# telegraphroad/VCNF

Measured on AMD Instinct MI355X. Metric: flow transforms/sec (log_prob + sample), D=64 RQ-spline, batch=1M, higher is better.
Workload: dtype f32 results on fp16x3 split operands: every fp32 operand of a conditioner GEMM travels as hi + lo fp16 halves, three f16 matrix instructions per product (four in the 48- and 16-deep layers), fp32 accumulation; measured against fp64 (tests/test_gpu_gemm_error.py): GEMM error 0.6-0.75x the exact-fp32

## Files before the change

vcnf_amd/csrc/fused_layer_v6.hip:

```cpp
#include <hip/hip_runtime.h>
#include <stdint.h>

#include "../../include/vcnf_hip.h"
#include "rqs_math.hpp"
#include "fused_common.hpp"
#include "rqs_lean.hpp"
#include "split_half.hpp"

#ifndef VCNF_ABL
#define VCNF_ABL 0
#endif
#ifndef VCNF_TIME
#define VCNF_TIME 0
#endif
#ifndef VCNF_AHEAD
#define VCNF_AHEAD 1
#endif
#if VCNF_TIME
#define VCNF_T(I) { const long long t_ = clock64(); tacc[I] += t_ - tlast; tlast = t_; }
#define VCNF_TIME_PARAM , float* tstamps
#define VCNF_TIME_ARG , time_buffer()
#else
#define VCNF_T(I)
#define VCNF_TIME_PARAM
#define VCNF_TIME_ARG
#endif

#define VCNF_SYNC() { __builtin_amdgcn_sched_barrier(0); asm volatile("s_waitcnt lgkmcnt(0)\n\ts_barrier" ::: "memory"); __builtin_amdgcn_sched_barrier(0); }

namespace vcnf {

#if VCNF_TIME
constexpr int kTimeSlots = 24;
static float* time_buffer() {
  static float* buf = nullptr;
  if (!buf && hipMalloc(&buf, 2 * kTimeSlots * sizeof(float)) != hipSuccess) buf = nullptr;
  return buf;
}
extern "C" int vcnf_v6_phase_stamps(float* out) {
  if (!time_buffer() || hipDeviceSynchronize() != hipSuccess) return VCNF_ERR_LAUNCH;
  return hipMemcpy(out, time_buffer(), 2 * kTimeSlots * sizeof(float), hipMemcpyDeviceToHost) == hipSuccess ? VCNF_OK : VCNF_ERR_LAUNCH;
}
#endif

template <int DI, int DT, int C, int H, int NBLK, int K, bool INV>
__global__ __launch_bounds__(512, 2) void fused_rqs_layer_v6_kernel(const FusedArgs a VCNF_TIME_PARAM) {
  static_assert(H == 128 && K == 8, "4 row blocks of 32 over 4 waves; 3 K - 1 = 23 logits: two features per 48 rows");
  static_assert((DI == 16 || DI == 32) && DT == DI && (C == 0 || C == 16), "shape family");
  constexpr int kBlock = 512;
  constexpr int kTile = 128;
  constexpr int NCB = 4;
  constexpr int D = DI + DT;
  constexpr int XS = D + 4;
  constexpr int NTX = DI / 16;
  constexpr int NTC = C / 16;
  constexpr int NT0 = NTX + NTC;
  constexpr int NTH = H / 16;
  constexpr int P = 3 * K - 1;
  constexpr int NG = DT / 4;
  constexpr int NR = NG / 2;
  constexpr int TABW = 3 * (K + 1);
  using L = PackLayout6<DI, DT, C, H, NBLK, K>;
  constexpr int GFRAG = 3 * NTH * 2 * 64;
  constexpr int RING = VCNF_AHEAD + 1;

  extern __shared__ __align__(16) float smem[];
  uint4* act = reinterpret_cast<uint4*>(smem);
  uint4* act_hi = act;
  uint4* act_lo = act + NTH * NCB * 64;
  float* xt = smem + 2 * GFRAG * 4;
  uint4* ctxf = reinterpret_cast<uint4*>(xt + kTile * XS);
  float* tab = reinterpret_cast<float*>(ctxf + (C > 0 ? NCB * 2 * 64 : 0));
  float* ldt = tab + ((DI * TABW + 3) & ~3);
  int* tfi = reinterpret_cast<int*>(ldt + kTile);
  int* idi = tfi + DT;
  constexpr int NBV = C > 0 ? 3 : 2;
  constexpr int NBT = 1 + NBLK * NBV;
  constexpr int BPL = NG * 48 + NBT * (H / 2);
  float* biasf = reinterpret_cast<float*>(idi + DI + 4);
  float* ldold = biasf + 2 * BPL;
  int* tflag = reinterpret_cast<int*>(ldold + kTile);

  const int tid = threadIdx.x;
  const int lane = tid & 63;
  const int wave = __builtin_amdgcn_readfirstlane(tid >> 6);
  const int rp = wave & 3;
  const int ch = wave >> 2;
  const int c32 = lane & 31;
  const int kg = lane >> 5;
  const RqsConst& c = a.c;
  const bool shared = a.sh_w != nullptr;
  const LeanConst lc = make_lean_const(c);

  if (ch == 1) __builtin_amdgcn_s_setprio(1);
  for (int i = tid; i < NG * 96; i += kBlock) {
    const int g = i / 96, hf = i % 96 / 48;
    biasf[hf * BPL + g * 48 + i % 48] = a.wpack[L::BF + i];
  }
  for (int i = tid; i < NBT * H; i += kBlock) {
    const int v = i / H, blk = (v - 1) / NBV, sel = (v - 1) % NBV, r = i % H;
    const int off = v == 0 ? L::B0 : L::BLK0 + blk * L::BLK + (sel == 0 ? L::BA : sel == 1 ? L::BB : L::BC);
    biasf[(r >> 4 & 1) * BPL + NG * 48 + v * (H / 2) + (r >> 5) * 16 + (r & 15)] = a.wpack[off + r];
  }
  for (int i = tid; i < DT; i += kBlock) tfi[i] = a.tf_idx[i];
  for (int i = tid; i < DI; i += kBlock) idi[i] = a.id_idx[i];
  if (shared) {
    for (int i = tid; i < 3 * DI; i += kBlock) {
      const int f = i % DI;
      SplitLogits p{a.sh_w + f * K, a.sh_h + f * K, a.sh_d + f * (K - 1), K, 1.f, c.edge_logit, c.tails};
      rqs_build_table_part_k<K>(p, c, tab + f * TABW, 1, i / DI);
    }
  }

  const __amdgpu_buffer_rsrc_t wr =
      __builtin_amdgcn_make_buffer_rsrc(const_cast<float*>(a.wpack), 0, a.wpack_bytes, 0x00020000);
  const int voff = lane * 16;
  const float* bplane = biasf + kg * BPL;

  const long long ntiles = (a.B + kTile - 1) / kTile;
  bool bad = false;
  float satm = 0.f;
#if VCNF_TIME
  long long tacc[20], tlast = clock64();
  const long long tstart = tlast, rstart = wall_clock64();
  for (int i = 0; i < 20; ++i) tacc[i] = 0;
#endif
  float4 xpre[kTile * (D / 4) / kBlock], cpre[1];
  static_assert(kTile * (D / 4) % kBlock == 0 && (C == 0 || kTile * (C / 4) == kBlock), "rows per thread");
#define VCNF_PREFETCH_ROWS(TILE)                                                          \
  {                                                                                       \
    const long long pb0 = min((TILE) * kTile, a.B);                                       \
    const long long left = (a.B - pb0) * (D * 4);                                         \
    const __amdgpu_buffer_rsrc_t xr_ = __builtin_amdgcn_make_buffer_rsrc(                 \
        const_cast<float*>(a.x) + pb0 * D, 0, (int)min(left, (long long)(kTile * D * 4)), 0x00020000); \
    _Pragma("unroll") for (int k = 0; k < kTile * (D / 4) / kBlock; ++k)                  \
      xpre[k] = __builtin_bit_cast(float4, __builtin_amdgcn_raw_buffer_load_b128(xr_, (tid + kBlock * k) * 16, 0, 0)); \
    if (C > 0) {                                                                          \
      const long long leftc = (a.B - pb0) * (C * 4);                                      \
      const __amdgpu_buffer_rsrc_t cr_ = __builtin_amdgcn_make_buffer_rsrc(               \
          const_cast<float*>(a.ctx) + pb0 * C, 0, (int)min(leftc, (long long)(kTile * C * 4)), 0x00020000); \
      cpre[0] = __builtin_bit_cast(float4, __builtin_amdgcn_raw_buffer_load_b128(cr_, tid * 16, 0, 0)); \
    }                                                                                     \
  }
#define VCNF_ROWS_ARRIVED()                                                               \
  {                                                                                       \
    _Pragma("unroll") for (int k = 0; k < kTile * (D / 4) / kBlock; ++k) {                \
      floatx4 v_ = __builtin_bit_cast(floatx4, xpre[k]);                                  \
      asm volatile("" : "+v"(v_));                                                        \
      xpre[k] = __builtin_bit_cast(float4, v_);                                           \
    }                                                                                     \
    if (C > 0) {                                                                          \
      floatx4 v_ = __builtin_bit_cast(floatx4, cpre[0]);                                  \
      asm volatile("" : "+v"(v_));                                                        \
      cpre[0] = __builtin_bit_cast(float4, v_);                                           \
    }                                                                                     \
  }
  VCNF_PREFETCH_ROWS((long long)blockIdx.x)
  VCNF_ROWS_ARRIVED()
  for (long long tile = blockIdx.x; tile < ntiles; tile += gridDim.x) {
    const long long b0 = tile * kTile;
    const int rows = (int)min((long long)kTile, a.B - b0);
    satm = 0.f;
    { VCNF_T(0) VCNF_SYNC(); VCNF_T(15) }
    {
      constexpr int D4 = D / 4;
      if (tid == 0) *tflag = 0;
#pragma unroll
      for (int k = 0; k < kTile * D4 / kBlock; ++k) {
        const int i = tid + kBlock * k;
        const int r = i / D4, o = i - r * D4;
        *reinterpret_cast<float4*>(xt + r * XS + 4 * o) = xpre[k];
      }
      if (C > 0) {
        const int r = tid >> 2, part = tid & 3;
        half4 h4, l4;
        const float cv[4] = {cpre[0].x, cpre[0].y, cpre[0].z, cpre[0].w};
#pragma unroll
        for (int i = 0; i < 4; ++i) satm = fmaxf(satm, cv[i] == cv[i] ? __builtin_fabsf(cv[i]) : __builtin_inff());
        asm volatile("" : "+v"(satm));
#pragma unroll
        for (int i = 0; i < 4; ++i) {
          const float x = __builtin_amdgcn_fmed3f(cv[i], -65504.f, 65504.f);
          const _Float16 hv = (_Float16)x;
          h4[i] = hv;
          l4[i] = (_Float16)((x - (float)hv) * kLoScale);
        }
        const int at = (((r >> 5) * 2) * 64 + (r & 31) + 32 * (part >> 1));
        uint2* dh = reinterpret_cast<uint2*>(ctxf + at) + (part & 1);
        uint2* dl = reinterpret_cast<uint2*>(ctxf + at + 64) + (part & 1);
        *dh = __builtin_bit_cast(uint2, h4);
        *dl = __builtin_bit_cast(uint2, l4);
      }
    }
    { VCNF_T(1) VCNF_SYNC(); VCNF_T(15) }

    {
      constexpr int UNR = DI / 4;
      const int mi = tid >> 2, part = tid & 3;
      float lsum = 0.f;
      float xv[UNR], fv[UNR];
      float* px[UNR];
#pragma unroll
      for (int k = 0; k < UNR; ++k) {
        px[k] = xt + mi * XS + idi[part * UNR + k];
        xv[k] = *px[k];
        fv[k] = xv[k];
      }
      if (shared) {
        float yv[UNR], lad[UNR];
        bool in_[UNR];
#pragma unroll
        for (int k = 0; k < UNR; ++k) {
          in_[k] = (xv[k] >= c.lo_x) && (xv[k] <= c.hi_x);
          bool bad1 = false;
          rqs_point_table_inside<INV, K>(in_[k] ? xv[k] : c.lo_x, tab + (part * UNR + k) * TABW, yv[k], lad[k], bad1);
          bad = bad || (bad1 && in_[k]);
        }
#pragma unroll
        for (int k = 0; k < UNR; ++k) {
          const float o = in_[k] ? yv[k] : xv[k];
          *px[k] = o;
          if (INV) fv[k] = o;
          lsum += in_[k] ? lad[k] : 0.f;
        }
      }
      lsum += __shfl_xor(lsum, 1, 64);
      lsum += __shfl_xor(lsum, 2, 64);
      int tid_ = tid;
      asm volatile("" : "+v"(tid_));
      if (part == 0) ldt[tid_ >> 2] = lsum;
#pragma unroll
      for (int k = 0; k < UNR; ++k) satm = fmaxf(satm, fv[k] == fv[k] ? 0.f : __builtin_inff());
      const int k0 = part * UNR;
      const int t0 = k0 >> 4, kg0 = (k0 >> 3) & 1;
      const int at = (t0 * NCB + (mi >> 5)) * 64 + (mi & 31) + 32 * kg0;
      if (UNR == 8) {
        half8 h8, l8;
        float f8[8];
#pragma unroll
        for (int k = 0; k < 8; ++k) f8[k] = fv[k < UNR ? k : 0];
        split8<false>(f8, h8, l8, satm);
        act_hi[at] = __builtin_bit_cast(uint4, h8);
        act_lo[at] = __builtin_bit_cast(uint4, l8);
      } else {
        half4 h4, l4;
        satm = fmaxf(fmaxf(satm, __builtin_fabsf(fv[0])), __builtin_fabsf(fv[1]));
        satm = fmaxf(fmaxf(satm, __builtin_fabsf(fv[2 < UNR ? 2 : 0])), __builtin_fabsf(fv[3 < UNR ? 3 : 0]));
        asm volatile("" : "+v"(satm));
#pragma unroll
        for (int i = 0; i < 4; ++i) {
          const float x = __builtin_amdgcn_fmed3f(fv[i < UNR ? i : 0], -65504.f, 65504.f);
          const _Float16 hv = (_Float16)x;
          h4[i] = hv;
          l4[i] = (_Float16)((x - (float)hv) * kLoScale);
        }
        reinterpret_cast<uint2*>(act_hi + at)[(k0 >> 2) & 1] = __builtin_bit_cast(uint2, h4);
        reinterpret_cast<uint2*>(act_lo + at)[(k0 >> 2) & 1] = __builtin_bit_cast(uint2, l4);
      }
    }
    { VCNF_T(2) VCNF_SYNC(); VCNF_T(15) }
    if (ch == 1) { VCNF_T(14) VCNF_SYNC(); VCNF_T(16) }

    half8 ahi[NTH], alo[NTH];
    floatx16 abias;
#define VCNF_LOAD_BIAS16(DST, VEC)                                                        \
  _Pragma("unroll") for (int i_ = 0; i_ < 4; ++i_) {                                      \
    const floatx4 b4_ = *reinterpret_cast<const floatx4*>(bplane + NG * 48 + (VEC) * (H / 2) + 16 * rp + 4 * i_); \
    DST[4 * i_ + 0] = b4_[0]; DST[4 * i_ + 1] = b4_[1]; DST[4 * i_ + 2] = b4_[2]; DST[4 * i_ + 3] = b4_[3]; \
  }
#define VCNF_LOAD_HIDDEN(WOFF, BVEC)                                                      \
  {                                                                                       \
    _Pragma("unroll") for (int t = 0; t < NTH; ++t) {                                     \
      ahi[t] = __builtin_bit_cast(half8, wload(wr, voff, 4 * ((WOFF) + ((rp * NTH + t) * 2 + 0) * 256))); \
      alo[t] = __builtin_bit_cast(half8, wload(wr, voff, 4 * ((WOFF) + ((rp * NTH + t) * 2 + 1) * 256))); \
    }                                                                                     \
    VCNF_LOAD_BIAS16(abias, BVEC)                                                         \
  }

    floatx16 h[2];
    {
      half8 w0h[NT0], w0l[NT0];
      floatx16 bias0;
#pragma unroll
      for (int t = 0; t < NT0; ++t) {
        w0h[t] = __builtin_bit_cast(half8, wload(wr, voff, 4 * (L::W0 + ((rp * NT0 + t) * 2 + 0) * 256)));
        w0l[t] = __builtin_bit_cast(half8, wload(wr, voff, 4 * (L::W0 + ((rp * NT0 + t) * 2 + 1) * 256)));
      }
      VCNF_LOAD_BIAS16(bias0, 0)
#pragma unroll
      for (int j = 0; j < 2; ++j) {
        const int cb = 2 * ch + j;
        floatx16 mainv = bias0, corr = {}, corr2 = {};
#pragma unroll
        for (int t = 0; t < NT0; ++t) {
          const half8 bh = __builtin_bit_cast(half8, t < NTX ? act_hi[(t * NCB + cb) * 64 + lane] : ctxf[(cb * 2 + 0) * 64 + lane]);
          const half8 bl = __builtin_bit_cast(half8, t < NTX ? act_lo[(t * NCB + cb) * 64 + lane] : ctxf[(cb * 2 + 1) * 64 + lane]);
          mainv = mfma32h(w0h[t], bh, mainv);
          corr = mfma32h(w0h[t], bl, corr);
          corr = mfma32h(w0l[t], bh, corr);
          corr2 = mfma32h(w0l[t], bl, corr2);
        }
#pragma unroll
        for (int r = 0; r < 16; ++r) h[j][r] = fmaf(fmaf(corr2[r], kLoUnscale, corr[r]), kLoUnscale, mainv[r]);
      }
    }
    { VCNF_T(3) VCNF_SYNC(); VCNF_T(15) }
#define VCNF_PUBLISH(SRC, RELU)                                                           \
  _Pragma("unroll") for (int j = 0; j < 2; ++j) {                                         \
    _Pragma("unroll") for (int hh = 0; hh < 2; ++hh) {                                    \
      float v8_[8];                                                                       \
      _Pragma("unroll") for (int i = 0; i < 8; ++i) v8_[i] = SRC[j][8 * hh + i];          \
      half8 h8_, l8_;                                                                     \
      split8<RELU>(v8_, h8_, l8_, satm);                                                  \
      const int at = ((2 * rp + hh) * NCB + 2 * ch + j) * 64 + lane;                      \
      act_hi[at] = __builtin_bit_cast(uint4, h8_);                                        \
      act_lo[at] = __builtin_bit_cast(uint4, l8_);                                        \
    }                                                                                     \
  }
    VCNF_LOAD_HIDDEN(L::BLK0 + L::WA, 1)
    VCNF_PUBLISH(h, true)
    { VCNF_T(4) VCNF_SYNC(); VCNF_T(15) }

#define VCNF_READ_B(T)                                                                    \
  {                                                                                       \
    rh[(T) % RING] = __builtin_bit_cast(half8, act_hi[((((T) & 7)) * NCB + 2 * ch + ((T) >> 3)) * 64 + lane]); \
    rl[(T) % RING] = __builtin_bit_cast(half8, act_lo[((((T) & 7)) * NCB + 2 * ch + ((T) >> 3)) * 64 + lane]); \
  }
#define VCNF_HIDDEN_COMPUTE(OUT)                                                          \
  {                                                                                       \
    half8 rh[RING], rl[RING];                 \
    floatx16 corr;                                                                        \
    _Pragma("unroll") for (int st_ = 0; st_ < VCNF_AHEAD; ++st_) {                        \
      VCNF_READ_B(st_)                                                                    \
    }                                                                                     \
    _Pragma("unroll") for (int st_ = 0; st_ < 2 * NTH; ++st_) {                           \
      const int j = st_ >> 3, tk_ = st_ & 7;                                              \
      if (st_ + VCNF_AHEAD < 2 * NTH) {                                                   \
        VCNF_READ_B(st_ + VCNF_AHEAD)                                                     \
      }                                                                                   \
      if (tk_ == 0) {                                                                       \
        OUT[j] = abias;                                                                   \
        corr = floatx16{};                                                                \
      }                                                                                   \
      OUT[j] = mfma32h(ahi[tk_], rh[st_ % RING], OUT[j]);                                      \
      corr = mfma32h(ahi[tk_], rl[st_ % RING], corr);                                          \
      corr = mfma32h(alo[tk_], rh[st_ % RING], corr);                                          \
      if (tk_ == NTH - 1) {                                                                 \
        _Pragma("unroll") for (int r = 0; r < 16; ++r) OUT[j][r] = fmaf(corr[r], kLoUnscale, OUT[j][r]); \
      }                                                                                   \
    }                                                                                     \
    __builtin_amdgcn_sched_group_barrier(0x100, 2 * VCNF_AHEAD, 0);                       \
    _Pragma("unroll") for (int st_ = 0; st_ + VCNF_AHEAD < 2 * NTH; ++st_) {              \
      __builtin_amdgcn_sched_group_barrier(0x100, 2, 0);                                  \
      __builtin_amdgcn_sched_group_barrier(0x008, 3, 0);                                  \
    }                                                                                     \
    __builtin_amdgcn_sched_group_barrier(0x008, 3 * VCNF_AHEAD, 0);                       \
  }

#pragma unroll
    for (int blk = 0; blk < (VCNF_ABL == 5 ? 0 : NBLK); ++blk) {
      const int base = L::BLK0 + blk * L::BLK;
      floatx16 t[2];
      VCNF_HIDDEN_COMPUTE(t)
      { VCNF_T(5) VCNF_SYNC(); VCNF_T(15) }
      VCNF_LOAD_HIDDEN(base + L::WB, 2 + blk * NBV)
      half8 wch, wcl;
      floatx16 gate[2], gbias;
      if (C > 0) {
        wch = __builtin_bit_cast(half8, wload(wr, voff, 4 * (base + L::WC + (rp * 2 + 0) * 256)));
        wcl = __builtin_bit_cast(half8, wload(wr, voff, 4 * (base + L::WC + (rp * 2 + 1) * 256)));
        VCNF_LOAD_BIAS16(gbias, 3 + blk * NBV)
      }
      VCNF_PUBLISH(t, true)
      { VCNF_T(6) VCNF_SYNC(); VCNF_T(15) }
      VCNF_HIDDEN_COMPUTE(t)
      if (C > 0 && VCNF_ABL != 6) {
#pragma unroll
        for (int j = 0; j < 2; ++j) {
          const half8 bh = __builtin_bit_cast(half8, ctxf[((2 * ch + j) * 2 + 0) * 64 + lane]);
          const half8 bl = __builtin_bit_cast(half8, ctxf[((2 * ch + j) * 2 + 1) * 64 + lane]);
          floatx16 corr = {}, corr2 = {};
          gate[j] = mfma32h(wch, bh, gbias);
          corr = mfma32h(wch, bl, corr);
          corr = mfma32h(wcl, bh, corr);
          corr2 = mfma32h(wcl, bl, corr2);
#pragma unroll
          for (int r = 0; r < 16; ++r) gate[j][r] = fmaf(fmaf(corr2[r], kLoUnscale, corr[r]), kLoUnscale, gate[j][r]);
        }
      }
      { VCNF_T(5) VCNF_SYNC(); VCNF_T(15) }
      if (blk + 1 < NBLK) {
        VCNF_LOAD_HIDDEN(base + L::BLK + L::WA, 1 + (blk + 1) * NBV)
      }
      if (C > 0 && VCNF_ABL != 6) {
#pragma unroll
        for (int j = 0; j < 2; ++j) {
#pragma unroll
          for (int r = 0; r < 16; ++r) {
            const float sg = hw_rcp(1.f + hw_exp2(-gate[j][r]));
            h[j][r] = fmaf(t[j][r], sg, h[j][r]);
          }
        }
      } else {
#pragma unroll
        for (int j = 0; j < 2; ++j) h[j] += t[j];
      }
      if (blk + 1 < NBLK) {
        VCNF_PUBLISH(h, true)
      } else {
        VCNF_PUBLISH(h, false)
      }
      { VCNF_T(7) VCNF_SYNC(); VCNF_T(15) }
    }
    if (ch == 0) { VCNF_T(14) VCNF_SYNC(); VCNF_T(17) }
#undef VCNF_HIDDEN_COMPUTE
#undef VCNF_READ_B
#undef VCNF_LOAD_HIDDEN
#undef VCNF_PUBLISH

    half8 fhi[NTH], flo[NTH];
#pragma unroll
    for (int t = 0; t < NTH; ++t) {
      fhi[t] = __builtin_bit_cast(half8, act_hi[(t * NCB + rp) * 64 + lane]);
      flo[t] = __builtin_bit_cast(half8, act_lo[(t * NCB + rp) * 64 + lane]);
    }
    float ld_acc = 0.f;
    uint4* win = act + ch * GFRAG;
    const int gtid = tid & 255;
    constexpr int NSTG = GFRAG / 256;
    static_assert(GFRAG % 256 == 0, "whole fragments per thread");
#define VCNF_STAGE_DMA(G)                                                                 \
  _Pragma("unroll") for (int k = 0; k < NSTG; ++k)                                        \
    dma16_to_lds(wr, win + (gtid & ~63) + k * 256, gtid * 16, 4 * (L::WF + (G) * (4 * GFRAG) + k * 1024));
    floatx16 pa[3];
#define VCNF_LOAD_BIASF(G)                                                                \
  _Pragma("unroll") for (int b = 0; b < 3; ++b) {                                         \
    _Pragma("unroll") for (int i_ = 0; i_ < 4; ++i_) {                                    \
      const floatx4 b4_ = *reinterpret_cast<const floatx4*>(bplane + (G) * 48 + 16 * b + 4 * i_); \
      pa[b][4 * i_ + 0] = b4_[0]; pa[b][4 * i_ + 1] = b4_[1]; pa[b][4 * i_ + 2] = b4_[2]; pa[b][4 * i_ + 3] = b4_[3]; \
    }                                                                                     \
  }
    VCNF_LOAD_BIASF(ch)
    { VCNF_T(8) VCNF_SYNC(); VCNF_T(15) }
    VCNF_STAGE_DMA(ch)
    if (ch == 0 && rp < 2 && a.ld_mode) {
      const __amdgpu_buffer_rsrc_t or_ = __builtin_amdgcn_make_buffer_rsrc(a.logdet + b0, 0, rows * 4, 0x00020000);
      __builtin_amdgcn_raw_ptr_buffer_load_lds(or_, (__attribute__((address_space(3))) void*)(ldold + rp * 64), 4,
                                               lane * 4, rp * 256, 0, 0);
    }
    wait_vector_memory();
    { VCNF_T(9) VCNF_SYNC(); VCNF_T(15) }
    if (ch == 1) { VCNF_T(14) VCNF_SYNC(); VCNF_T(18) }
    for (int rnd = 0; rnd < (VCNF_ABL == 3 ? 0 : NR); ++rnd) {
      const int g = 2 * rnd + ch;
      float* px[2];
      float xin[2];
#pragma unroll
      for (int f2 = 0; f2 < 2; ++f2) {
        px[f2] = xt + (rp * 32 + c32) * XS + tfi[4 * g + 2 * kg + f2];
        xin[f2] = *px[f2];
      }
      {
        half8 wh[RING], wl[RING];
        floatx16 corr;
#define VCNF_READ_W(T)                                                                    \
  {                                                                                       \
    wh[(T) % RING] = __builtin_bit_cast(half8, win[((T) * 2 + 0) * 64 + lane]);           \
    wl[(T) % RING] = __builtin_bit_cast(half8, win[((T) * 2 + 1) * 64 + lane]);           \
  }
#pragma unroll
        for (int u = 0; u < VCNF_AHEAD; ++u) {
          VCNF_READ_W(u)
        }
#pragma unroll
        for (int u = 0; u < 3 * NTH; ++u) {
          const int b = u >> 3, t = u & 7;
          if (u + VCNF_AHEAD < 3 * NTH) {
            VCNF_READ_W(u + VCNF_AHEAD)
          }
          if (t == 0) corr = floatx16{};
          pa[b] = mfma32h(wh[u % RING], fhi[t], pa[b]);
          corr = mfma32h(wh[u % RING], flo[t], corr);
          corr = mfma32h(wl[u % RING], fhi[t], corr);
          if (t == NTH - 1) {
#pragma unroll
            for (int r = 0; r < 16; ++r) pa[b][r] = fmaf(corr[r], kLoUnscale, pa[b][r]);
          }
        }
        __builtin_amdgcn_sched_group_barrier(0x100, 2 * VCNF_AHEAD, 0);
#pragma unroll
        for (int u = 0; u + VCNF_AHEAD < 3 * NTH; ++u) {
          __builtin_amdgcn_sched_group_barrier(0x100, 2, 0);
          __builtin_amdgcn_sched_group_barrier(0x008, 3, 0);
        }
        __builtin_amdgcn_sched_group_barrier(0x008, 3 * VCNF_AHEAD, 0);
#undef VCNF_READ_W
      }
      { VCNF_T(10) VCNF_SYNC(); VCNF_T(15) }
      {
        const bool more = rnd + 1 < NR;
        if (!more) {
          VCNF_PREFETCH_ROWS(tile + gridDim.x)
        }
        if (more && VCNF_ABL != 2) {
          VCNF_STAGE_DMA(g + 2)
        }
        float yv[2], lad[2];
#pragma unroll
        for (int f2 = 0; f2 < 2; ++f2) {
          float lg[P];
#pragma unroll
          for (int tl = 0; tl < P; ++tl) lg[tl] = pa[(24 * f2 + tl) >> 4][(24 * f2 + tl) & 15];
          rqs_lean_eval<8, INV>(xin[f2], lg, lc, yv[f2], lad[f2], bad);
        }
        *px[0] = yv[0];
        *px[1] = yv[1];
        ld_acc += lad[0] + lad[1];
        if (more) {
          VCNF_LOAD_BIASF(g + 2)
        }
      }
      if (rnd + 1 < NR && VCNF_ABL != 2) wait_vector_memory();
      { VCNF_T(11) VCNF_SYNC(); VCNF_T(15) }
    }
    if (ch == 0) { VCNF_T(14) VCNF_SYNC(); VCNF_T(19) }
#undef VCNF_PREFETCH_ROWS
#undef VCNF_STAGE_DMA
#undef VCNF_LOAD_BIASF

    ld_acc += __shfl_xor(ld_acc, 32, 64);
    if (ch == 1 && kg == 0) ldt[rp * 32 + c32] += ld_acc;
    if (satm > 65504.f) *tflag = 1;
    { VCNF_T(12) VCNF_SYNC(); VCNF_T(15) }
    VCNF_ROWS_ARRIVED()
#undef VCNF_ROWS_ARRIVED
    int tid_ = tid;
    asm volatile("" : "+v"(tid_));
    const bool over = *tflag != 0;
    if (tid == 0 && over && a.sat) atomicAdd(a.sat, 1);
    if (a.redo) {
      if (tid_ < kTile / kFusedFlagRows) {
        const __amdgpu_buffer_rsrc_t rr = __builtin_amdgcn_make_buffer_rsrc(
            a.redo + tile * (kTile / kFusedFlagRows), 0, 4 * ((rows + kFusedFlagRows - 1) / kFusedFlagRows), 0x00020000);
        __builtin_amdgcn_raw_buffer_store_b32(over ? 1 : 0, rr, tid_ * 4, 0, 0);
      }
      if (over) continue;
    }
    if (ch == 0 && (tid_ & 32) == 0) {
      const int mrow = (tid_ >> 6) * 32 + (tid_ & 31);
      const __amdgpu_buffer_rsrc_t lr = __builtin_amdgcn_make_buffer_rsrc(a.logdet + b0, 0, rows * 4, 0x00020000);
      const float o = a.ld_sign * (ld_acc + ldt[mrow]);
      __builtin_amdgcn_raw_buffer_store_b32(__builtin_bit_cast(unsigned, a.ld_mode ? ldold[mrow] + o : o), lr, mrow * 4, 0, 0);
    }
    {
      constexpr int D4 = D / 4;
      const __amdgpu_buffer_rsrc_t yr = __builtin_amdgcn_make_buffer_rsrc(a.y + b0 * D, 0, rows * (D * 4), 0x00020000);
      floatx4 yv[kTile * D4 / kBlock];
#pragma unroll
      for (int k = 0; k < kTile * D4 / kBlock; ++k) {
        const int i = tid_ + kBlock * k;
        const int r = i / D4, o = i - r * D4;
        yv[k] = *reinterpret_cast<const floatx4*>(xt + r * XS + 4 * o);
      }
#pragma unroll
      for (int k = 0; k < kTile * D4 / kBlock; ++k)
        __builtin_amdgcn_raw_buffer_store_b128(__builtin_bit_cast(__attribute__((ext_vector_type(4))) unsigned, yv[k]), yr, (tid_ + kBlock * k) * 16, 0, 0);
    }
  }
#if VCNF_TIME
  VCNF_T(13)
  if (blockIdx.x == 0 && (tid & 255) == 0 && tstamps) {
    float* ts = tstamps + (tid >> 8) * kTimeSlots;
    for (int i = 0; i < 20; ++i) ts[i] = (float)tacc[i];
    ts[20] = (float)(clock64() - tstart);
    ts[21] = (float)(wall_clock64() - rstart);
    ts[22] = (float)((ntiles - blockIdx.x + gridDim.x - 1) / gridDim.x);
  }
#endif
  if (INV && a.bad && bad) atomicAdd(a.bad, 1);
}

template <int DI, int DT, int C, int H, int NBLK, int K>
static int launch_v6(const FusedArgs& a, int inverse, hipStream_t st) {
  constexpr int D = DI + DT;
  constexpr int TILE = 128;
  constexpr size_t WIN = (size_t)2 * 3 * (H / 16) * 2 * 64 * 16;
  constexpr int NBT = 1 + NBLK * (C > 0 ? 3 : 2);
  const size_t lds = ((size_t)TILE * (D + 4) + ((DI * 3 * (K + 1) + 3) & ~3) + 2 * TILE + D + 8 + (DT / 4) * 96 + NBT * H) * 4 +
                     (C > 0 ? 4 * 2 * 64 * 16 : 0) + WIN + 64;
  static bool attr_set[2] = {false, false};
  if (!attr_set[inverse ? 1 : 0]) {
    hipError_t e;
    if (inverse)
      e = hipFuncSetAttribute(reinterpret_cast<const void*>(&fused_rqs_layer_v6_kernel<DI, DT, C, H, NBLK, K, true>),
                              hipFuncAttributeMaxDynamicSharedMemorySize, (int)lds);
    else
      e = hipFuncSetAttribute(reinterpret_cast<const void*>(&fused_rqs_layer_v6_kernel<DI, DT, C, H, NBLK, K, false>),
                              hipFuncAttributeMaxDynamicSharedMemorySize, (int)lds);
    if (e != hipSuccess) return VCNF_ERR_LAUNCH;
    attr_set[inverse ? 1 : 0] = true;
  }
  const long long ntiles = (a.B + TILE - 1) / TILE;
  dim3 grid((unsigned)(ntiles < 256 ? ntiles : 256));
  if (inverse)
    hipLaunchKernelGGL((fused_rqs_layer_v6_kernel<DI, DT, C, H, NBLK, K, true>), grid, dim3(512), lds, st, a VCNF_TIME_ARG);
  else
    hipLaunchKernelGGL((fused_rqs_layer_v6_kernel<DI, DT, C, H, NBLK, K, false>), grid, dim3(512), lds, st, a VCNF_TIME_ARG);
  return hipGetLastError() == hipSuccess ? VCNF_OK : VCNF_ERR_LAUNCH;
}

template <int NBLK>
static int launch_v6_family(const FusedArgs& a, int d_id, int ctx_dim, int inverse, hipStream_t st) {
#ifdef VCNF_DEV_ONLY
  return launch_v6<32, 32, 16, 128, NBLK, 8>(a, inverse, st);
#else
  if (d_id == 32) {
    return ctx_dim == 16 ? launch_v6<32, 32, 16, 128, NBLK, 8>(a, inverse, st)
                         : launch_v6<32, 32, 0, 128, NBLK, 8>(a, inverse, st);
  }
  return ctx_dim == 16 ? launch_v6<16, 16, 16, 128, NBLK, 8>(a, inverse, st)
                       : launch_v6<16, 16, 0, 128, NBLK, 8>(a, inverse, st);
#endif
}

#ifndef VCNF_V6_NBLK
#define VCNF_V6_NBLK 2
#endif
#if VCNF_V6_NBLK == 1
int launch_fused_v6_b1(const FusedArgs& a, int d_id, int ctx_dim, int inverse, hipStream_t st) {
  return launch_v6_family<1>(a, d_id, ctx_dim, inverse, st);
}
#elif VCNF_V6_NBLK == 2
int launch_fused_v6_b2(const FusedArgs& a, int d_id, int ctx_dim, int inverse, hipStream_t st) {
  return launch_v6_family<2>(a, d_id, ctx_dim, inverse, st);
}
#else
int launch_fused_v6_b3(const FusedArgs& a, int d_id, int ctx_dim, int inverse, hipStream_t st) {
  return launch_v6_family<3>(a, d_id, ctx_dim, inverse, st);
}
#endif

}
```

Baseline: 73.68 million.

## Hand-schedule split-fp16 MFMA chains with explicit fences and cross-block overlap

Replaces the ring-buffered LDS operand reads and sched_group_barrier hints in the hidden-layer, input-layer and output-layer split-fp16 GEMMs with fully unrolled per-step register arrays and explicit sched_barrier fences. At block boundaries the next block's main MFMAs are interleaved with the previous block's correction FMA, and the context gate GEMM and its bias load are folded into the tail of the hidden compute. The output rounds are turned into a lambda with the last round peeled for one shape, and several tid/lane values are pinned through asm to keep the address math in VGPRs. The aim is to hide MFMA dependency latency and LDS latency, at the cost of more register pressure and a rigid hand-written schedule.

```diff
diff --git a/vcnf_amd/csrc/fused_layer_v6.hip b/vcnf_amd/csrc/fused_layer_v6.hip
--- a/vcnf_amd/csrc/fused_layer_v6.hip
+++ b/vcnf_amd/csrc/fused_layer_v6.hip
@@ -1,5 +1,6 @@
 #include <hip/hip_runtime.h>
 #include <stdint.h>
+#include <type_traits>
 
 #include "../../include/vcnf_hip.h"
 #include "rqs_math.hpp"
@@ -28,7 +29,12 @@
 
 #define VCNF_SYNC() { __builtin_amdgcn_sched_barrier(0); asm volatile("s_waitcnt lgkmcnt(0)\n\ts_barrier" ::: "memory"); __builtin_amdgcn_sched_barrier(0); }
 
+#define VCNF_FENCE() __builtin_amdgcn_sched_barrier(0)
+
 namespace vcnf {
+
+__device__ constexpr bool ho_first(int u) { return (u & 7) == 0 && u > 0; }
+__device__ constexpr bool ho_second(int u) { return (u & 7) == 1 && u > 8; }
 
 #if VCNF_TIME
 constexpr int kTimeSlots = 24;
@@ -62,7 +68,6 @@
   constexpr int TABW = 3 * (K + 1);
   using L = PackLayout6<DI, DT, C, H, NBLK, K>;
   constexpr int GFRAG = 3 * NTH * 2 * 64;
-  constexpr int RING = VCNF_AHEAD + 1;
 
   extern __shared__ __align__(16) float smem[];
   uint4* act = reinterpret_cast<uint4*>(smem);
@@ -129,17 +134,19 @@
   static_assert(kTile * (D / 4) % kBlock == 0 && (C == 0 || kTile * (C / 4) == kBlock), "rows per thread");
 #define VCNF_PREFETCH_ROWS(TILE)                                                          \
   {                                                                                       \
+    int ptid_ = tid;                            \
+    asm volatile("" : "+v"(ptid_));                                                       \
     const long long pb0 = min((TILE) * kTile, a.B);                                       \
     const long long left = (a.B - pb0) * (D * 4);                                         \
     const __amdgpu_buffer_rsrc_t xr_ = __builtin_amdgcn_make_buffer_rsrc(                 \
         const_cast<float*>(a.x) + pb0 * D, 0, (int)min(left, (long long)(kTile * D * 4)), 0x00020000); \
     _Pragma("unroll") for (int k = 0; k < kTile * (D / 4) / kBlock; ++k)                  \
-      xpre[k] = __builtin_bit_cast(float4, __builtin_amdgcn_raw_buffer_load_b128(xr_, (tid + kBlock * k) * 16, 0, 0)); \
+      xpre[k] = __builtin_bit_cast(float4, __builtin_amdgcn_raw_buffer_load_b128(xr_, (ptid_ + kBlock * k) * 16, 0, 0)); \
     if (C > 0) {                                                                          \
       const long long leftc = (a.B - pb0) * (C * 4);                                      \
       const __amdgpu_buffer_rsrc_t cr_ = __builtin_amdgcn_make_buffer_rsrc(               \
           const_cast<float*>(a.ctx) + pb0 * C, 0, (int)min(leftc, (long long)(kTile * C * 4)), 0x00020000); \
-      cpre[0] = __builtin_bit_cast(float4, __builtin_amdgcn_raw_buffer_load_b128(cr_, tid * 16, 0, 0)); \
+      cpre[0] = __builtin_bit_cast(float4, __builtin_amdgcn_raw_buffer_load_b128(cr_, ptid_ * 16, 0, 0)); \
     }                                                                                     \
   }
 #define VCNF_ROWS_ARRIVED()                                                               \
@@ -165,14 +172,16 @@
     {
       constexpr int D4 = D / 4;
       if (tid == 0) *tflag = 0;
+      int tidc = tid;
+      asm volatile("" : "+v"(tidc));
 #pragma unroll
       for (int k = 0; k < kTile * D4 / kBlock; ++k) {
-        const int i = tid + kBlock * k;
+        const int i = tidc + kBlock * k;
         const int r = i / D4, o = i - r * D4;
         *reinterpret_cast<float4*>(xt + r * XS + 4 * o) = xpre[k];
       }
       if (C > 0) {
-        const int r = tid >> 2, part = tid & 3;
+        const int r = tidc >> 2, part = tidc & 3;
         half4 h4, l4;
         const float cv[4] = {cpre[0].x, cpre[0].y, cpre[0].z, cpre[0].w};
 #pragma unroll
@@ -287,21 +296,41 @@
         w0l[t] = __builtin_bit_cast(half8, wload(wr, voff, 4 * (L::W0 + ((rp * NT0 + t) * 2 + 1) * 256)));
       }
       VCNF_LOAD_BIAS16(bias0, 0)
+      half8 bh[2][NT0], bl[2][NT0];
+      int lane0 = lane;
+      asm volatile("" : "+v"(lane0));
 #pragma unroll
       for (int j = 0; j < 2; ++j) {
         const int cb = 2 * ch + j;
-        floatx16 mainv = bias0, corr = {}, corr2 = {};
 #pragma unroll
         for (int t = 0; t < NT0; ++t) {
-          const half8 bh = __builtin_bit_cast(half8, t < NTX ? act_hi[(t * NCB + cb) * 64 + lane] : ctxf[(cb * 2 + 0) * 64 + lane]);
-          const half8 bl = __builtin_bit_cast(half8, t < NTX ? act_lo[(t * NCB + cb) * 64 + lane] : ctxf[(cb * 2 + 1) * 64 + lane]);
-          mainv = mfma32h(w0h[t], bh, mainv);
-          corr = mfma32h(w0h[t], bl, corr);
-          corr = mfma32h(w0l[t], bh, corr);
-          corr2 = mfma32h(w0l[t], bl, corr2);
-        }
-#pragma unroll
-        for (int r = 0; r < 16; ++r) h[j][r] = fmaf(fmaf(corr2[r], kLoUnscale, corr[r]), kLoUnscale, mainv[r]);
+          bh[j][t] = __builtin_bit_cast(half8, t < NTX ? act_hi[(t * NCB + cb) * 64 + lane0] : ctxf[(cb * 2 + 0) * 64 + lane0]);
+          bl[j][t] = __builtin_bit_cast(half8, t < NTX ? act_lo[(t * NCB + cb) * 64 + lane0] : ctxf[(cb * 2 + 1) * 64 + lane0]);
+        }
+      }
+      VCNF_FENCE();
+      constexpr int NA0 = NT0 < 2 ? NT0 : 2;
+      floatx16 mainv[2] = {bias0, bias0}, corr, corr2;
+#pragma unroll
+      for (int j = 0; j < 2; ++j) {
+        corr = floatx16{};
+        corr2 = floatx16{};
+#pragma unroll
+        for (int t = 0; t < NT0; ++t) {
+          if (j == 0 || t >= NA0) mainv[j] = mfma32h(w0h[t], bh[j][t], mainv[j]);
+          corr = mfma32h(w0h[t], bl[j][t], corr);
+          corr = mfma32h(w0l[t], bh[j][t], corr);
+          corr2 = mfma32h(w0l[t], bl[j][t], corr2);
+          VCNF_FENCE();
+        }
+        if (j == 0) {
+#pragma unroll
+          for (int t = 0; t < NA0; ++t) mainv[1] = mfma32h(w0h[t], bh[1][t], mainv[1]);
+          VCNF_FENCE();
+        }
+#pragma unroll
+        for (int r = 0; r < 16; ++r) h[j][r] = fmaf(fmaf(corr2[r], kLoUnscale, corr[r]), kLoUnscale, mainv[j][r]);
+        VCNF_FENCE();
       }
     }
     { VCNF_T(3) VCNF_SYNC(); VCNF_T(15) }
@@ -321,73 +350,105 @@
     VCNF_PUBLISH(h, true)
     { VCNF_T(4) VCNF_SYNC(); VCNF_T(15) }
 
-#define VCNF_READ_B(T)                                                                    \
+#define VCNF_RH(X) rh[X] = __builtin_bit_cast(half8, act_hi[(((X) & 7) * NCB + 2 * ch + ((X) >> 3)) * 64 + lane]);
+#define VCNF_RL(X) rl[X] = __builtin_bit_cast(half8, act_lo[(((X) & 7) * NCB + 2 * ch + ((X) >> 3)) * 64 + lane]);
+#define VCNF_CORR_FMA(DST) _Pragma("unroll") for (int r = 0; r < 16; ++r) DST[r] = fmaf(corr[r], kLoUnscale, DST[r]);
+#define VCNF_HIDDEN_COMPUTE(OUT, GATE, GVEC)                                                  \
   {                                                                                       \
-    rh[(T) % RING] = __builtin_bit_cast(half8, act_hi[((((T) & 7)) * NCB + 2 * ch + ((T) >> 3)) * 64 + lane]); \
-    rl[(T) % RING] = __builtin_bit_cast(half8, act_lo[((((T) & 7)) * NCB + 2 * ch + ((T) >> 3)) * 64 + lane]); \
-  }
-#define VCNF_HIDDEN_COMPUTE(OUT)                                                          \
-  {                                                                                       \
-    half8 rh[RING], rl[RING];                 \
+    constexpr int U_ = 2 * NTH, A_ = VCNF_AHEAD;                                          \
+    half8 rh[U_], rl[U_];                            \
     floatx16 corr;                                                                        \
-    _Pragma("unroll") for (int st_ = 0; st_ < VCNF_AHEAD; ++st_) {                        \
-      VCNF_READ_B(st_)                                                                    \
-    }                                                                                     \
-    _Pragma("unroll") for (int st_ = 0; st_ < 2 * NTH; ++st_) {                           \
-      const int j = st_ >> 3, tk_ = st_ & 7;                                              \
-      if (st_ + VCNF_AHEAD < 2 * NTH) {                                                   \
-        VCNF_READ_B(st_ + VCNF_AHEAD)                                                     \
+    _Pragma("unroll") for (int x = 0; x < U_; ++x) {                                      \
+      if (x - (ho_second(x) ? 1 : 0) < A_) { VCNF_RH(x) }                                 \
+      if (x < A_) { VCNF_RL(x) }                                                          \
+    }                                                                                     \
+    OUT[0] = abias;                                                                       \
+    OUT[1] = abias;                                                                       \
+    VCNF_FENCE();                                                                         \
+    _Pragma("unroll") for (int st_ = 0; st_ < U_; ++st_) {                                \
+      const int tk_ = st_ & 7;                                                            \
+      _Pragma("unroll") for (int x = st_ + A_; x <= st_ + A_ + 1 && x < U_; ++x) {        \
+        if (x - (ho_second(x) ? 1 : 0) - A_ == st_) { VCNF_RH(x) }                        \
+        if (x - A_ == st_ && !ho_first(x) && !ho_second(st_)) { VCNF_RL(x) }              \
       }                                                                                   \
-      if (tk_ == 0) {                                                                       \
-        OUT[j] = abias;                                                                   \
-        corr = floatx16{};                                                                \
+      if ((GATE) && st_ == U_ - 2) {                                                      \
+        VCNF_LOAD_BIAS16(gbias, GVEC)                                                     \
       }                                                                                   \
-      OUT[j] = mfma32h(ahi[tk_], rh[st_ % RING], OUT[j]);                                      \
-      corr = mfma32h(ahi[tk_], rl[st_ % RING], corr);                                          \
-      corr = mfma32h(alo[tk_], rh[st_ % RING], corr);                                          \
-      if (tk_ == NTH - 1) {                                                                 \
-        _Pragma("unroll") for (int r = 0; r < 16; ++r) OUT[j][r] = fmaf(corr[r], kLoUnscale, OUT[j][r]); \
+      if ((GATE) && st_ == U_ - 1) {                                                      \
+        _Pragma("unroll") for (int j = 0; j < 2; ++j) {                                   \
+          gbh[j] = __builtin_bit_cast(half8, ctxf[((2 * ch + j) * 2 + 0) * 64 + lane]);   \
+          gbl[j] = __builtin_bit_cast(half8, ctxf[((2 * ch + j) * 2 + 1) * 64 + lane]);   \
+        }                                                                                 \
       }                                                                                   \
-    }                                                                                     \
-    __builtin_amdgcn_sched_group_barrier(0x100, 2 * VCNF_AHEAD, 0);                       \
-    _Pragma("unroll") for (int st_ = 0; st_ + VCNF_AHEAD < 2 * NTH; ++st_) {              \
-      __builtin_amdgcn_sched_group_barrier(0x100, 2, 0);                                  \
-      __builtin_amdgcn_sched_group_barrier(0x008, 3, 0);                                  \
-    }                                                                                     \
-    __builtin_amdgcn_sched_group_barrier(0x008, 3 * VCNF_AHEAD, 0);                       \
+      VCNF_FENCE();                                                                       \
+      if (ho_first(st_)) {                                                                \
+        OUT[1] = mfma32h(ahi[0], rh[st_], OUT[1]);                                        \
+        OUT[1] = mfma32h(ahi[1], rh[st_ + 1], OUT[1]);                                    \
+        VCNF_FENCE();                                                                     \
+        VCNF_CORR_FMA(OUT[0])                                                             \
+        VCNF_FENCE();                                                                     \
+        corr = mfma32h(ahi[0], rl[st_], floatx16{});                                      \
+      } else if (ho_second(st_)) {                                                        \
+        corr = mfma32h(alo[0], rh[st_ - 1], corr);                                        \
+        VCNF_FENCE();                                                                     \
+        if (st_ + A_ < U_) { VCNF_RL(st_ + A_) }                                          \
+        VCNF_FENCE();                                                                     \
+        corr = mfma32h(ahi[1], rl[st_], corr);                                            \
+        corr = mfma32h(alo[1], rh[st_], corr);                                            \
+      } else {                                                                            \
+        OUT[st_ >> 3] = mfma32h(ahi[tk_], rh[st_], OUT[st_ >> 3]);                        \
+        corr = mfma32h(ahi[tk_], rl[st_], tk_ == 0 ? floatx16{} : corr);                  \
+        VCNF_FENCE();                                                                     \
+        if (st_ + A_ < U_ && ho_first(st_ + A_)) { VCNF_RL(st_ + A_) }                    \
+        VCNF_FENCE();                                                                     \
+        corr = mfma32h(alo[tk_], rh[st_], corr);                                          \
+      }                                                                                   \
+      VCNF_FENCE();                                                                       \
+    }                                                                                     \
+    if (!(GATE)) {                                                                        \
+      VCNF_CORR_FMA(OUT[1])                                                               \
+    } else {                                                                              \
+       \
+       \
+       \
+       \
+                                                          \
+      floatx16 gc[2], gc2[2];                                                             \
+      gate[0] = mfma32h(wch, gbh[0], gbias);                                              \
+      gate[1] = mfma32h(wch, gbh[1], gbias);                                              \
+      VCNF_FENCE();                                                                       \
+      VCNF_CORR_FMA(OUT[1])                                                               \
+      VCNF_FENCE();                                                                       \
+      gc[0] = mfma32h(wch, gbl[0], floatx16{});                                           \
+      gc[0] = mfma32h(wcl, gbh[0], gc[0]);                                                \
+      gc2[0] = mfma32h(wcl, gbl[0], floatx16{});                                          \
+      gc[1] = mfma32h(wch, gbl[1], floatx16{});                                           \
+      gc[1] = mfma32h(wcl, gbh[1], gc[1]);                                                \
+      VCNF_FENCE();                                                                       \
+      _Pragma("unroll") for (int r = 0; r < 16; ++r) gate[0][r] = fmaf(fmaf(gc2[0][r], kLoUnscale, gc[0][r]), kLoUnscale, gate[0][r]); \
+      VCNF_FENCE();                                                                       \
+      gc2[1] = mfma32h(wcl, gbl[1], floatx16{});                                          \
+      VCNF_FENCE();                                                                       \
+      _Pragma("unroll") for (int r = 0; r < 16; ++r) gate[1][r] = fmaf(fmaf(gc2[1][r], kLoUnscale, gc[1][r]), kLoUnscale, gate[1][r]); \
+    }                                                                                     \
   }
 
 #pragma unroll
     for (int blk = 0; blk < (VCNF_ABL == 5 ? 0 : NBLK); ++blk) {
       const int base = L::BLK0 + blk * L::BLK;
       floatx16 t[2];
-      VCNF_HIDDEN_COMPUTE(t)
+      half8 wch, wcl, gbh[2], gbl[2];
+      floatx16 gate[2], gbias;
+      VCNF_HIDDEN_COMPUTE(t, false, 0)
       { VCNF_T(5) VCNF_SYNC(); VCNF_T(15) }
       VCNF_LOAD_HIDDEN(base + L::WB, 2 + blk * NBV)
-      half8 wch, wcl;
-      floatx16 gate[2], gbias;
       if (C > 0) {
         wch = __builtin_bit_cast(half8, wload(wr, voff, 4 * (base + L::WC + (rp * 2 + 0) * 256)));
         wcl = __builtin_bit_cast(half8, wload(wr, voff, 4 * (base + L::WC + (rp * 2 + 1) * 256)));
-        VCNF_LOAD_BIAS16(gbias, 3 + blk * NBV)
       }
       VCNF_PUBLISH(t, true)
       { VCNF_T(6) VCNF_SYNC(); VCNF_T(15) }
-      VCNF_HIDDEN_COMPUTE(t)
-      if (C > 0 && VCNF_ABL != 6) {
-#pragma unroll
-        for (int j = 0; j < 2; ++j) {
-          const half8 bh = __builtin_bit_cast(half8, ctxf[((2 * ch + j) * 2 + 0) * 64 + lane]);
-          const half8 bl = __builtin_bit_cast(half8, ctxf[((2 * ch + j) * 2 + 1) * 64 + lane]);
-          floatx16 corr = {}, corr2 = {};
-          gate[j] = mfma32h(wch, bh, gbias);
-          corr = mfma32h(wch, bl, corr);
-          corr = mfma32h(wcl, bh, corr);
-          corr2 = mfma32h(wcl, bl, corr2);
-#pragma unroll
-          for (int r = 0; r < 16; ++r) gate[j][r] = fmaf(fmaf(corr2[r], kLoUnscale, corr[r]), kLoUnscale, gate[j][r]);
-        }
-      }
+      VCNF_HIDDEN_COMPUTE(t, C > 0 && VCNF_ABL != 6, 3 + blk * NBV)
       { VCNF_T(5) VCNF_SYNC(); VCNF_T(15) }
       if (blk + 1 < NBLK) {
         VCNF_LOAD_HIDDEN(base + L::BLK + L::WA, 1 + (blk + 1) * NBV)
@@ -414,7 +475,8 @@
     }
     if (ch == 0) { VCNF_T(14) VCNF_SYNC(); VCNF_T(17) }
 #undef VCNF_HIDDEN_COMPUTE
-#undef VCNF_READ_B
+#undef VCNF_RH
+#undef VCNF_RL
 #undef VCNF_LOAD_HIDDEN
 #undef VCNF_PUBLISH
 
@@ -445,60 +507,84 @@
     VCNF_STAGE_DMA(ch)
     if (ch == 0 && rp < 2 && a.ld_mode) {
       const __amdgpu_buffer_rsrc_t or_ = __builtin_amdgcn_make_buffer_rsrc(a.logdet + b0, 0, rows * 4, 0x00020000);
+      int lane_ = lane;
+      asm volatile("" : "+v"(lane_));
       __builtin_amdgcn_raw_ptr_buffer_load_lds(or_, (__attribute__((address_space(3))) void*)(ldold + rp * 64), 4,
-                                               lane * 4, rp * 256, 0, 0);
+                                               lane_ * 4, rp * 256, 0, 0);
     }
     wait_vector_memory();
     { VCNF_T(9) VCNF_SYNC(); VCNF_T(15) }
     if (ch == 1) { VCNF_T(14) VCNF_SYNC(); VCNF_T(18) }
-    for (int rnd = 0; rnd < (VCNF_ABL == 3 ? 0 : NR); ++rnd) {
+    constexpr bool kPeelLastRound = DI == 32 && C == 16;
+    auto round_steps = [&](const int rnd, auto more_) __attribute__((always_inline)) {
+      const bool more = more_;
       const int g = 2 * rnd + ch;
       float* px[2];
       float xin[2];
-#pragma unroll
-      for (int f2 = 0; f2 < 2; ++f2) {
-        px[f2] = xt + (rp * 32 + c32) * XS + tfi[4 * g + 2 * kg + f2];
-        xin[f2] = *px[f2];
-      }
       {
-        half8 wh[RING], wl[RING];
+        constexpr int U = 3 * NTH, A = VCNF_AHEAD;
+        half8 wh[U], wl[U];
         floatx16 corr;
-#define VCNF_READ_W(T)                                                                    \
-  {                                                                                       \
-    wh[(T) % RING] = __builtin_bit_cast(half8, win[((T) * 2 + 0) * 64 + lane]);           \
-    wl[(T) % RING] = __builtin_bit_cast(half8, win[((T) * 2 + 1) * 64 + lane]);           \
-  }
-#pragma unroll
-        for (int u = 0; u < VCNF_AHEAD; ++u) {
-          VCNF_READ_W(u)
-        }
-#pragma unroll
-        for (int u = 0; u < 3 * NTH; ++u) {
+        int fi[2];
+#define VCNF_WH(X) wh[X] = __builtin_bit_cast(half8, win[((X) * 2 + 0) * 64 + lane]);
+#define VCNF_WL(X) wl[X] = __builtin_bit_cast(half8, win[((X) * 2 + 1) * 64 + lane]);
+#pragma unroll
+        for (int x = 0; x < U; ++x) {
+          if (x - (ho_second(x) ? 1 : 0) < A) { VCNF_WH(x) }
+          if (x + (ho_first(x) ? 1 : 0) < A) { VCNF_WL(x) }
+        }
+        VCNF_FENCE();
+#pragma unroll
+        for (int u = 0; u < U; ++u) {
           const int b = u >> 3, t = u & 7;
-          if (u + VCNF_AHEAD < 3 * NTH) {
-            VCNF_READ_W(u + VCNF_AHEAD)
+#pragma unroll
+          for (int x = u + A - 1; x <= u + A + 1 && x < U; ++x) {
+            if (x - (ho_second(x) ? 1 : 0) - A == u) { VCNF_WH(x) }
+            if (x + (ho_first(x) ? 1 : 0) - A == u && !ho_second(u)) { VCNF_WL(x) }
           }
-          if (t == 0) corr = floatx16{};
-          pa[b] = mfma32h(wh[u % RING], fhi[t], pa[b]);
-          corr = mfma32h(wh[u % RING], flo[t], corr);
-          corr = mfma32h(wl[u % RING], fhi[t], corr);
-          if (t == NTH - 1) {
-#pragma unroll
-            for (int r = 0; r < 16; ++r) pa[b][r] = fmaf(corr[r], kLoUnscale, pa[b][r]);
+          if (u == U - 1) {
+            int kg_ = kg;
+            asm volatile("" : "+v"(kg_));
+#pragma unroll
+            for (int f2 = 0; f2 < 2; ++f2) fi[f2] = tfi[4 * g + 2 * kg_ + f2];
           }
-        }
-        __builtin_amdgcn_sched_group_barrier(0x100, 2 * VCNF_AHEAD, 0);
-#pragma unroll
-        for (int u = 0; u + VCNF_AHEAD < 3 * NTH; ++u) {
-          __builtin_amdgcn_sched_group_barrier(0x100, 2, 0);
-          __builtin_amdgcn_sched_group_barrier(0x008, 3, 0);
-        }
-        __builtin_amdgcn_sched_group_barrier(0x008, 3 * VCNF_AHEAD, 0);
-#undef VCNF_READ_W
+          VCNF_FENCE();
+          if (ho_first(u)) {
+            pa[b] = mfma32h(wh[u], fhi[0], pa[b]);
+            pa[b] = mfma32h(wh[u + 1], fhi[1], pa[b]);
+            VCNF_FENCE();
+            VCNF_CORR_FMA(pa[b - 1])
+            VCNF_FENCE();
+            corr = mfma32h(wh[u], flo[0], floatx16{});
+          } else if (ho_second(u)) {
+            corr = mfma32h(wl[u - 1], fhi[0], corr);
+            VCNF_FENCE();
+#pragma unroll
+            for (int x = u + A - 1; x <= u + A && x < U; ++x) {
+              if (x + (ho_first(x) ? 1 : 0) - A == u) { VCNF_WL(x) }
+            }
+            VCNF_FENCE();
+            corr = mfma32h(wh[u], flo[1], corr);
+            corr = mfma32h(wl[u], fhi[1], corr);
+          } else {
+            pa[b] = mfma32h(wh[u], fhi[t], pa[b]);
+            corr = mfma32h(wh[u], flo[t], t == 0 ? floatx16{} : corr);
+            corr = mfma32h(wl[u], fhi[t], corr);
+          }
+          VCNF_FENCE();
+        }
+        VCNF_CORR_FMA(pa[2])
+        VCNF_FENCE();
+#pragma unroll
+        for (int f2 = 0; f2 < 2; ++f2) {
+          px[f2] = xt + (rp * 32 + c32) * XS + fi[f2];
+          xin[f2] = *px[f2];
+        }
+#undef VCNF_WH
+#undef VCNF_WL
       }
       { VCNF_T(10) VCNF_SYNC(); VCNF_T(15) }
       {
-        const bool more = rnd + 1 < NR;
         if (!more) {
           VCNF_PREFETCH_ROWS(tile + gridDim.x)
         }
@@ -520,16 +606,27 @@
           VCNF_LOAD_BIASF(g + 2)
         }
       }
-      if (rnd + 1 < NR && VCNF_ABL != 2) wait_vector_memory();
+      if (more && VCNF_ABL != 2) wait_vector_memory();
       { VCNF_T(11) VCNF_SYNC(); VCNF_T(15) }
+    };
+    if (kPeelLastRound) {
+      for (int rnd = 0; rnd < (VCNF_ABL == 3 ? 0 : NR - 1); ++rnd) round_steps(rnd, std::true_type{});
+      if (VCNF_ABL != 3) round_steps(NR - 1, std::false_type{});
+    } else {
+      for (int rnd = 0; rnd < (VCNF_ABL == 3 ? 0 : NR); ++rnd) round_steps(rnd, rnd + 1 < NR);
     }
     if (ch == 0) { VCNF_T(14) VCNF_SYNC(); VCNF_T(19) }
+#undef VCNF_CORR_FMA
 #undef VCNF_PREFETCH_ROWS
 #undef VCNF_STAGE_DMA
 #undef VCNF_LOAD_BIASF
 
     ld_acc += __shfl_xor(ld_acc, 32, 64);
-    if (ch == 1 && kg == 0) ldt[rp * 32 + c32] += ld_acc;
+    {
+      int lane_ = lane;
+      asm volatile("" : "+v"(lane_));
+      if (ch == 1 && lane_ < 32) ldt[rp * 32 + lane_] += ld_acc;
+    }
     if (satm > 65504.f) *tflag = 1;
     { VCNF_T(12) VCNF_SYNC(); VCNF_T(15) }
     VCNF_ROWS_ARRIVED()
```

Result: no change. 74.33 million (median of 6 runs) (+0.9%).
